# Human-Augment-Analytics/vectordb-retrieval

Measured on AMD Instinct MI355X. Metric: QPS @ recall@10 (SIFT1M-shaped, 10k-query batch, k=10), higher is better.
Workload: dtype i8 MFMA scan (i32 accumulate) + exact integer / f64 refine

## Files before the change

### vectordb-retrieval_amd/csrc/scan_i8x16.hpp

```cpp
#pragma once
#include "scan_i8.hpp"

namespace vdb {

__host__ __device__ inline int x16_row_in_span(int t, int rb, int m) { return (m >> 2) * 128 + t * 8 + rb * 4 + (m & 3); }

__device__ __forceinline__ int swap16(int v) { return __builtin_amdgcn_ds_swizzle(v, 0x401F); }

template <int KS2, int ST, int RING>
constexpr int scan_i8x16_lds_bytes() { return RING * (ST * 2 * KS2 * 64 * 16 + ST * 32 * 4); }

template <int N_MFMA, int N_VALU, int N_DS>
__device__ __forceinline__ void x16_gap_pattern() {
    constexpr int R = (N_VALU + N_DS + N_MFMA - 1) / N_MFMA;
    static_assert(N_DS <= N_MFMA && R >= 2, "one LDS read per gap");
#pragma unroll
    for (int i = 0; i < N_MFMA; ++i) {
        __builtin_amdgcn_sched_group_barrier(0x8, 1, 0);
        if (i < N_DS) {
            __builtin_amdgcn_sched_group_barrier(0x100, 1, 0);
            __builtin_amdgcn_sched_group_barrier(0x2, R - 1, 0);
        } else {
            __builtin_amdgcn_sched_group_barrier(0x2, R, 0);
        }
    }
}

template <int KS2, int ST, int CB, class StageIssue, class BiasStore, class FlushBin>
__device__ __forceinline__ void scan_i8x16_batch_loop(const unsigned char *smem, const int4v (&bq)[CB][KS2], int (&m1)[CB], int (&m2)[CB],
                                                      int nstages, int64_t span0, int lane, StageIssue &&stage_issue,
                                                      BiasStore &&stage_bias_store, FlushBin &&flush_bin) {
    constexpr int NV = 2 * KS2, kStageVec = ST * NV * 64, TPS = kTilesPerSpan, SPS = TPS / ST;
    constexpr int NM = 2 * KS2 * CB, NH = NM / 2;
    static_assert(ST % 2 == 0 && TPS % ST == 0, "tile parity must be static in the unrolled stage");
    const int g = lane >> 4;
    const unsigned id_hi = (g & 1) ? 16u : 0u;
    int4v acc[2][2][CB], fr[2][NV], cin[2][2];
    int q[CB];
#pragma unroll
    for (int rb = 0; rb < 2; ++rb)
#pragma unroll
        for (int cb = 0; cb < CB; ++cb)
#pragma unroll
            for (int r = 0; r < 4; ++r) acc[1][rb][cb][r] = (int)(kI8Inf >> 6);
    auto read_tile = [&](int p, const int4v *A, const int4v *B4, int t) {
#pragma unroll
        for (int v = 0; v < NV; ++v) fr[p][v] = A[(t * NV + v) * 64];
        cin[p][0] = B4[t * 8];
        cin[p][1] = B4[t * 8 + 1];
    };
    auto mfma_half = [&](int p, int half) {
#pragma unroll
        for (int m = half * NH; m < (half + 1) * NH; ++m) {
            const int ks = m / (2 * CB), rb = (m / CB) % 2, cb = m % CB;
            acc[p][rb][cb] = __builtin_amdgcn_mfma_i32_16x16x64_i8(fr[p][2 * ks + rb], bq[cb][ks], ks == 0 ? cin[p][rb] : acc[p][rb][cb], 0, 0, 0);
        }
    };
    auto min_trees = [&](int o) {
#pragma unroll
        for (int cb = 0; cb < CB; ++cb) {
            const int t1 = imin(imin(acc[o][0][cb][0], acc[o][0][cb][1]), acc[o][0][cb][2]);
            const int t2 = imin(imin(acc[o][0][cb][3], acc[o][1][cb][0]), acc[o][1][cb][1]);
            q[cb] = imin(imin(imin(acc[o][1][cb][2], acc[o][1][cb][3]), t1), t2);
        }
    };
    auto folds = [&](int t_bin) {
        const unsigned idv = (unsigned)__builtin_amdgcn_readfirstlane(t_bin) | id_hi;
#pragma unroll
        for (int cb = 0; cb < CB; ++cb) {
            const int v = (int)(((unsigned)q[cb] << 6) | idv);
            m2[cb] = imed3(m1[cb], m2[cb], v);
            m1[cb] = imin(m1[cb], v);
        }
    };
    for (int st = 0; st < nstages; ++st) {
        const int buf = st & 1;
        if (st + 1 < nstages) stage_issue(st + 1, buf ^ 1);
        const int4v *A = reinterpret_cast<const int4v *>(smem + buf * (kStageVec * 16)) + lane;
        const int4v *B4 = reinterpret_cast<const int4v *>(smem + 2 * kStageVec * 16 + buf * (ST * 32 * 4)) + g * 2;
        const int ts0 = (st % SPS) * ST;
        read_tile(0, A, B4, 0);
#pragma unroll
        for (int t = 0; t < ST; ++t) {
            const int p = t & 1, o = p ^ 1;
            __builtin_amdgcn_sched_barrier(0);
            mfma_half(p, 0);
            min_trees(o);
            x16_gap_pattern<NH, 4 * CB, 0>();
            __builtin_amdgcn_sched_barrier(0);
#pragma unroll
            for (int cb = 0; cb < CB; ++cb) asm volatile("" : "+v"(q[cb]));
            __builtin_amdgcn_sched_barrier(0);
            if (t + 1 < ST) read_tile(o, A, B4, t + 1);
            mfma_half(p, 1);
            folds((ts0 + t + TPS - 1) % TPS);
            x16_gap_pattern<NH, 3 * CB + 1, NV + 2>();
            __builtin_amdgcn_sched_barrier(0);
#pragma unroll
            for (int cb = 0; cb < CB; ++cb) asm volatile("" : "+v"(m1[cb]), "+v"(m2[cb]));
            if (t == 0 && st > 0 && ts0 == 0) flush_bin(span0 + st / SPS - 1);
        }
        __builtin_amdgcn_sched_barrier(0);
        if (st + 1 < nstages) stage_bias_store(buf ^ 1);
        __syncthreads();
    }
    min_trees((ST - 1) & 1);
    folds(TPS - 1);
    flush_bin(span0 + nstages / SPS - 1);
}

template <int KS2, int ST, int CB, int NWAVES = 8, int RING = 2, int AUX = 0>
__device__ __forceinline__ void scan_i8x16_body(const ScanI8Args &a, unsigned char *smem) {
    constexpr int NV = 2 * KS2;
    constexpr int NT = NWAVES * 64;
    constexpr int kStageVec = ST * NV * 64;
    constexpr int kBiasLoads = (ST * 32 + NT - 1) / NT;
    constexpr int TPS = kTilesPerSpan;
    constexpr int SPS = TPS / ST;
    constexpr int HC = CB / 2;
    constexpr int UNR = (ST * CB <= 16) ? ST : 1;
    static_assert(TPS % ST == 0 && ST >= 2 && CB % 2 == 0 && NWAVES <= 8, "bad geometry");
    static_assert(RING >= 2 && RING <= 8 && (RING == 2 || ST % 2 == 0), "bad ring");
    constexpr bool kDeep = RING > 2;
    static_assert(scan_i8x16_lds_bytes<KS2, ST, RING>() == RING * (kStageVec * 16 + ST * 32 * 4), "LDS size");
    const int mode = a.info->i8_mode;
    if (!mode) return;
    auto lds_a = [&](int buf) { return reinterpret_cast<int4v *>(smem + buf * (kStageVec * 16)); };
    auto lds_b = [&](int buf) { return reinterpret_cast<int *>(smem + RING * kStageVec * 16 + buf * (ST * 32 * 4)); };

    const int tid = threadIdx.x, lane = tid & 63;
    const int wave = __builtin_amdgcn_readfirstlane(tid >> 6);
    const int g = lane >> 4, h = g >> 1;
    const bool odd = (g & 1) != 0;
    const bool late = (NWAVES >= 2) && (wave >= NWAVES / 2);
    const int b = blockIdx.x;
    const int x = b & 7, jb = b >> 3;
    const int ci = jb / a.nqtiles, qt = jb - ci * a.nqtiles;
    const int chunk = x + 8 * ci;
    if (chunk >= a.nchunks) return;
    const int64_t q0 = (int64_t)qt * (NWAVES * 16 * CB) + wave * (16 * CB);
    const int64_t span0 = chunk_span0(chunk, a.spans_per_chunk, a.chunk_rem);
    int64_t span1 = chunk_span0(chunk + 1, a.spans_per_chunk, a.chunk_rem);
    if (span1 > a.nspans) span1 = a.nspans;
    const int64_t out_pitch = a.Qpad;
    const int64_t col0 = q0 + (odd ? 16 : 0) + (lane & 15);
    const int32_t *bias = a.bias8 + ((mode & 3) == 1 ? 0 : a.Npad);

    int4v bq[CB][KS2];
#pragma unroll
    for (int cb = 0; cb < CB; ++cb)
#pragma unroll
        for (int ks = 0; ks < KS2; ++ks) bq[cb][ks] = a.qpanels[((size_t)(q0 / 16 + cb) * KS2 + ks) * 64 + lane];
    const int nstages = (int)(span1 - span0) * SPS;
    const int INF = (int)kI8Inf;
    int m1[CB], m2[CB], M1[HC], M2[HC], Ms[HC];
#pragma unroll
    for (int cb = 0; cb < CB; ++cb) m1[cb] = m2[cb] = INF;
#pragma unroll
    for (int j = 0; j < HC; ++j) {
        M1[j] = M2[j] = INF;
        Ms[j] = 0;
    }

    constexpr int kPieces = kStageVec / 64;
    static_assert(kPieces % NWAVES == 0, "pieces must divide over the waves");
    constexpr int kBiasPieces = (ST / 2 + NWAVES - 1) / NWAVES;
    int stage_b[kBiasLoads];
    auto stage_issue = [&](int st, int buf) {
        const int64_t span = span0 + st / SPS;
        const int sq = st % SPS;
        const int4v *src = a.panels + ((size_t)(span * TPS + sq * ST) * NV) * 64;
        int4v *dst = lds_a(buf);
#pragma unroll
        for (int i = 0; i < kPieces / NWAVES; ++i) {
            const int p = wave + i * NWAVES;
            const int4v *gp = src + p * 64 + lane;
            __builtin_amdgcn_global_load_lds(
                reinterpret_cast<const __attribute__((address_space(1))) void *>(reinterpret_cast<uintptr_t>(gp)),
                reinterpret_cast<__attribute__((address_space(3))) void *>(
                    static_cast<uint32_t>(reinterpret_cast<uintptr_t>(dst + p * 64))),
                16, 0, AUX);
        }
        if (kDeep) {
#pragma unroll
            for (int i = 0; i < kBiasPieces; ++i) {
                const int j = (wave + i * NWAVES) % (ST / 2);
                const int t = 2 * j + (lane >> 5), gg = (lane >> 3) & 3, e = lane & 7;
                const int32_t *gp = bias + span * kSpanRows + gg * 128 + (sq * ST + t) * 8 + e;
                __builtin_amdgcn_global_load_lds(
                    reinterpret_cast<const __attribute__((address_space(1))) void *>(reinterpret_cast<uintptr_t>(gp)),
                    reinterpret_cast<__attribute__((address_space(3))) void *>(
                        static_cast<uint32_t>(reinterpret_cast<uintptr_t>(lds_b(buf) + j * 64))),
                    4, 0, 0);
            }
            return;
        }
#pragma unroll
        for (int i = 0; i < kBiasLoads; ++i) {
            const int e = tid + i * NT;
            if (e < ST * 32) {
                const int t = e >> 5, gg = (e >> 3) & 3, r = e & 7;
                stage_b[i] = bias[span * kSpanRows + gg * 128 + (sq * ST + t) * 8 + r];
            }
        }
    };
    auto stage_bias_store = [&](int buf) {
        if (kDeep) return;
#pragma unroll
        for (int i = 0; i < kBiasLoads; ++i)
            if (tid + i * NT < ST * 32) lds_b(buf)[tid + i * NT] = stage_b[i];
    };
    auto ring_issue = [&](int st) { stage_issue(st < nstages ? st : nstages - 1, st % RING); };
    auto ring_wait = [&]() {
        constexpr int kKeep = (RING - 2) * (kPieces / NWAVES + kBiasPieces);
        static_assert(kKeep < 64, "vmcnt is a 6-bit counter");
        asm volatile("s_waitcnt vmcnt(%0)" ::"n"(kKeep) : "memory");
        __builtin_amdgcn_s_barrier();
        asm volatile("" ::: "memory");
    };
    auto flush_bin = [&](int64_t span) {
        const size_t o = (size_t)(span * 2 + h) * out_pitch + col0;
#pragma unroll
        for (int j = 0; j < HC; ++j) {
            const int p1 = swap16(odd ? m1[2 * j] : m1[2 * j + 1]), p2 = swap16(odd ? m2[2 * j] : m2[2 * j + 1]);
            const int a1 = odd ? m1[2 * j + 1] : m1[2 * j], a2 = odd ? m2[2 * j + 1] : m2[2 * j];
            const int b1 = imin(a1, p1), b2 = imin(imax(a1, p1), imin(a2, p2));
            __builtin_nontemporal_store(__int_as_float(b1), a.bin_m1 + o + j * 32);
            __builtin_nontemporal_store(__int_as_float(b2), a.bin_m2 + o + j * 32);
            M2[j] = imin(imed3(M1[j], M2[j], b1), b2);
            if (b1 < M1[j]) Ms[j] = (int)span;
            M1[j] = imin(M1[j], b1);
        }
#pragma unroll
        for (int cb = 0; cb < CB; ++cb) m1[cb] = m2[cb] = INF;
    };

    if (kDeep) {
#pragma unroll
        for (int s = 0; s < RING - 1; ++s) ring_issue(s);
    } else {
        stage_issue(0, 0);
    }
    stage_bias_store(0);
    if (kDeep) ring_wait();
    else __syncthreads();

    if (a.nq_valid > 0 && q0 >= a.nq_valid) {
        for (int st = 0; st < nstages; ++st) {
            if (kDeep) {
                ring_issue(st + RING - 1);
                ring_wait();
                continue;
            }
            if (st + 1 < nstages) {
                stage_issue(st + 1, (st & 1) ^ 1);
                stage_bias_store((st & 1) ^ 1);
            }
            __syncthreads();
        }
        return;
    }

    if constexpr (NWAVES == 8 && RING == 2 && UNR == 1) {
        scan_i8x16_batch_loop<KS2, ST, CB>(smem, bq, m1, m2, nstages, span0, lane, stage_issue, stage_bias_store, flush_bin);
    } else {
    int4v fr[NV], cin[2], acc[2][CB];
    auto read_phase = [&](const int4v *A_tile, const int4v *c_tile) {
#pragma unroll
        for (int v = 0; v < NV; ++v) fr[v] = A_tile[v * 64 + lane];
        cin[0] = c_tile[0];
        cin[1] = c_tile[1];
    };
    auto mfma_phase = [&]() {
#pragma unroll
        for (int ks = 0; ks < KS2; ++ks)
#pragma unroll
            for (int rb = 0; rb < 2; ++rb)
#pragma unroll
                for (int cb = 0; cb < CB; ++cb)
                    acc[rb][cb] = __builtin_amdgcn_mfma_i32_16x16x64_i8(fr[2 * ks + rb], bq[cb][ks], ks == 0 ? cin[rb] : acc[rb][cb], 0, 0, 0);
    };
    const unsigned id_hi = odd ? 16u : 0u;
    auto select_phase = [&](int t_bin) {
        const unsigned idv = (unsigned)__builtin_amdgcn_readfirstlane(t_bin) | id_hi;
#pragma unroll
        for (int cb = 0; cb < CB; ++cb) {
            const int t1 = imin(imin(acc[0][cb][0], acc[0][cb][1]), acc[0][cb][2]);
            const int t2 = imin(imin(acc[0][cb][3], acc[1][cb][0]), acc[1][cb][1]);
            const int q = imin(imin(imin(acc[1][cb][2], acc[1][cb][3]), t1), t2);
            const int v = (int)(((unsigned)q << 6) | idv);
            m2[cb] = imed3(m1[cb], m2[cb], v);
            m1[cb] = imin(m1[cb], v);
        }
    };
    if (a.prio == 1 && late) __builtin_amdgcn_s_setprio(1);
    else if (a.prio == 2 && !late) __builtin_amdgcn_s_setprio(1);
    if (!late) {
        for (int st = 0; st < nstages; ++st) {
            const int buf = kDeep ? st % RING : st & 1;
            if (kDeep) ring_issue(st + RING - 1);
            else if (st + 1 < nstages) stage_issue(st + 1, buf ^ 1);
            const int4v *A = lds_a(buf);
            const int4v *B4 = reinterpret_cast<const int4v *>(lds_b(buf)) + g * 2;
            const int ts0 = (st % SPS) * ST;
            read_phase(A, B4);
#pragma unroll UNR
            for (int t = 0; t < ST; ++t) {
                __builtin_amdgcn_sched_barrier(0);
                mfma_phase();
                __builtin_amdgcn_sched_barrier(0);
                if (t + 1 < ST) read_phase(A + (t + 1) * NV * 64, B4 + (t + 1) * 8);
                select_phase(ts0 + t);
            }
            __builtin_amdgcn_sched_barrier(0);
            if (ts0 + ST == TPS) flush_bin(span0 + st / SPS);
            if (!kDeep && st + 1 < nstages) stage_bias_store(buf ^ 1);
            if (kDeep) ring_wait();
            else __syncthreads();
        }
    } else {
#pragma unroll
        for (int rb = 0; rb < 2; ++rb)
#pragma unroll
            for (int cb = 0; cb < CB; ++cb)
#pragma unroll
                for (int r = 0; r < 4; ++r) acc[rb][cb][r] = (int)(kI8Inf >> 6);
        for (int st = 0; st < nstages; ++st) {
            const int buf = kDeep ? st % RING : st & 1;
            if (kDeep) ring_issue(st + RING - 1);
            else if (st + 1 < nstages) stage_issue(st + 1, buf ^ 1);
            const int4v *A = lds_a(buf);
            const int4v *B4 = reinterpret_cast<const int4v *>(lds_b(buf)) + g * 2;
            const int ts0 = (st % SPS) * ST;
#pragma unroll UNR
            for (int t = 0; t < ST; ++t) {
                __builtin_amdgcn_sched_barrier(0);
                read_phase(A + t * NV * 64, B4 + t * 8);
                select_phase((ts0 + t + TPS - 1) % TPS);
                if (t == 0 && st > 0 && ts0 == 0) flush_bin(span0 + st / SPS - 1);
                __builtin_amdgcn_sched_barrier(0);
                mfma_phase();
            }
            __builtin_amdgcn_sched_barrier(0);
            if (!kDeep && st + 1 < nstages) stage_bias_store(buf ^ 1);
            if (kDeep) ring_wait();
            else __syncthreads();
        }
        select_phase(TPS - 1);
        flush_bin(span1 - 1);
    }
    }

    const size_t so = (size_t)(chunk * 2 + h) * a.Qpad + col0;
#pragma unroll
    for (int j = 0; j < HC; ++j) {
        a.sb_m1[so + j * 32] = __int_as_float(M1[j]);
        a.sb_m2[so + j * 32] = __int_as_float(M2[j]);
        a.sb_span[so + j * 32] = Ms[j];
    }
}

template <int KS2, int ST, int CB, int NWAVES = 8, int RING = 2, int AUX = 0>
__global__ __launch_bounds__(NWAVES * 64, (NWAVES >= 4 ? 2 : 1)) void scan_i8x16_kernel(ScanI8Args a) {
    __shared__ __attribute__((aligned(16))) unsigned char smem[scan_i8x16_lds_bytes<KS2, ST, RING>()];
    scan_i8x16_body<KS2, ST, CB, NWAVES, RING, AUX>(a, smem);
}

}
```

### vectordb-retrieval_amd/csrc/scan_x16.hpp

```cpp
#pragma once
#include "scan16.hpp"
#include "scan_i8x16.hpp"

namespace vdb {

template <int KS2, int ST>
constexpr int scan_x16_lds_bytes() { return 2 * (ST * 2 * KS2 * 64 * 16 + ST * 32 * 4); }

template <int KS2, int NWAVES, int ST, int BR = 256, int G = 8, int CB = 4>
__device__ __forceinline__ void scan_x16_body(const ScanArgs &a, unsigned char *smem) {
    constexpr int NV = 2 * KS2;
    static_assert(CB == 4 || (CB == 8 && KS2 <= 2), "128 queries per wave: D <= 64");
    constexpr int NT = NWAVES * 64;
    constexpr int kStageVec = ST * NV * 64;
    constexpr int kBiasLoads = (ST * 32 + NT - 1) / NT;
    constexpr int TPS = kTilesPerSpan;
    constexpr int SPS = TPS / ST;
    constexpr int BT = BR == 64 ? 8 : 16;
    constexpr bool kMerge = BR == 256;
    constexpr int NS = kMerge ? CB / 2 : CB;
    constexpr int UNR = ST <= 4 ? ST : 1;
    static_assert(TPS % ST == 0 && ST >= 2 && BT % ST == 0 && (BR == 256 || BR == 128 || BR == 64), "bad geometry");
    static_assert(G == 8 || (G == 4 && BR != 256), "quads: direct-bin mode");
    static_assert(scan_x16_lds_bytes<KS2, ST>() == 2 * (kStageVec * 16 + ST * 32 * 4), "LDS size");
    auto lds_a = [&](int buf) { return reinterpret_cast<half8 *>(smem + buf * (kStageVec * 16)); };
    auto lds_b = [&](int buf) { return reinterpret_cast<float *>(smem + 2 * kStageVec * 16 + buf * (ST * 32 * 4)); };
    if (a.info->i8_mode) return;

    const int tid = threadIdx.x, lane = tid & 63;
    const int wave = __builtin_amdgcn_readfirstlane(tid >> 6);
    const int g = lane >> 4, h = g >> 1;
    const bool odd = (g & 1) != 0;
    const bool late = (NWAVES >= 2) && (wave >= NWAVES / 2);
    const int b = blockIdx.x;
    const int x = b & 7, jb = b >> 3;
    const int ci = jb / a.nqtiles, qt = jb - ci * a.nqtiles;
    int chunk = x + 8 * ci;
    if (chunk >= a.nchunks) return;
    chunk += a.chunk0;
    const int64_t q0 = (int64_t)qt * (NWAVES * 16 * CB) + wave * (16 * CB);
    const int64_t span0 = chunk_span0(chunk, a.spans_per_chunk, a.chunk_rem);
    int64_t span1 = chunk_span0(chunk + 1, a.spans_per_chunk, a.chunk_rem);
    if (span1 > a.nspans) span1 = a.nspans;
    const int64_t col0 = q0 + ((kMerge && odd) ? 16 : 0) + (lane & 15);
    constexpr int CS = kMerge ? 32 : 16;
    const float cs = a.info->cs;

    half8 bq[CB][KS2];
#pragma unroll
    for (int cb = 0; cb < CB; ++cb)
#pragma unroll
        for (int ks = 0; ks < KS2; ++ks) bq[cb][ks] = a.qpanels[((size_t)(q0 / 16 + cb) * KS2 + ks) * 64 + lane];
    const int nstages = (int)(span1 - span0) * SPS;
    const float INF = __builtin_inff();
    float NEG_INF = -INF;
    asm volatile("" : "+v"(NEG_INF));
    unsigned idmask = kQuadIdMask;
    asm volatile("" : "+v"(idmask));
    float m1[CB], m2[CB], M1[NS], M2[NS];
    int Ms[NS];
#pragma unroll
    for (int cb = 0; cb < CB; ++cb) m1[cb] = m2[cb] = INF;
#pragma unroll
    for (int j = 0; j < NS; ++j) {
        M1[j] = M2[j] = INF;
        Ms[j] = 0;
    }

    constexpr int kPieces = kStageVec / 64;
    static_assert(kPieces % NWAVES == 0, "pieces must divide over the waves");
    float stage_b[kBiasLoads];
    auto stage_issue = [&](int st, int buf) {
        const int64_t span = span0 + st / SPS;
        const int sq = st % SPS;
        const half8 *src = a.panels + ((size_t)(span * TPS + sq * ST) * NV) * 64;
        half8 *dst = lds_a(buf);
#pragma unroll
        for (int i = 0; i < kPieces / NWAVES; ++i) {
            const int p = wave + i * NWAVES;
            const half8 *gp = src + p * 64 + lane;
            __builtin_amdgcn_global_load_lds(
                reinterpret_cast<const __attribute__((address_space(1))) void *>(reinterpret_cast<uintptr_t>(gp)),
                reinterpret_cast<__attribute__((address_space(3))) void *>(
                    static_cast<uint32_t>(reinterpret_cast<uintptr_t>(dst + p * 64))),
                16, 0, NWAVES <= 2 ? 2 : 0);
        }
#pragma unroll
        for (int i = 0; i < kBiasLoads; ++i) {
            const int e = tid + i * NT;
            if (e < ST * 32) {
                const int t = e >> 5, gg = (e >> 3) & 3, r = e & 7;
                stage_b[i] = a.bias[span * kSpanRows + gg * 128 + (sq * ST + t) * 8 + r];
            }
        }
    };
    auto stage_bias_store = [&](int buf) {
#pragma unroll
        for (int i = 0; i < kBiasLoads; ++i)
            if (tid + i * NT < ST * 32)
                lds_b(buf)[tid + i * NT] = (stage_b[i] >= 0.9e38f) ? kPadBias : stage_b[i] * cs;
    };
    auto flush_bin = [&](int64_t span, int bt) {
        if (kMerge) {
            const size_t o = (size_t)(span * 2 + h) * a.Qpad + col0;
#pragma unroll
            for (int j = 0; j < NS; ++j) {
                const float p1 = __int_as_float(swap16(__float_as_int(odd ? m1[2 * j] : m1[2 * j + 1])));
                const float p2 = __int_as_float(swap16(__float_as_int(odd ? m2[2 * j] : m2[2 * j + 1])));
                const float a1 = odd ? m1[2 * j + 1] : m1[2 * j], a2 = odd ? m2[2 * j + 1] : m2[2 * j];
                const float b1 = __builtin_fminf(a1, p1), b2 = __builtin_fminf(__builtin_fmaxf(a1, p1), __builtin_fminf(a2, p2));
                __builtin_nontemporal_store(b1, a.bin_m1 + o + j * CS);
                __builtin_nontemporal_store(b2, a.bin_m2 + o + j * CS);
                M2[j] = __builtin_fminf(__builtin_amdgcn_fmed3f(M1[j], M2[j], b1), b2);
                if (b1 < M1[j]) Ms[j] = (int)span;
                M1[j] = __builtin_fminf(M1[j], b1);
            }
        } else {
            const size_t o = (size_t)((span * 4 + g) * (128 / BR) + bt) * a.Qpad + col0;
#pragma unroll
            for (int j = 0; j < NS; ++j) {
                __builtin_nontemporal_store(m1[j], a.bin_m1 + o + j * 16);
                __builtin_nontemporal_store(m2[j], a.bin_m2 + o + j * 16);
                M2[j] = __builtin_fminf(__builtin_amdgcn_fmed3f(M1[j], M2[j], m1[j]), m2[j]);
                if (m1[j] < M1[j]) Ms[j] = (int)span;
                M1[j] = __builtin_fminf(M1[j], m1[j]);
            }
        }
#pragma unroll
        for (int cb = 0; cb < CB; ++cb) m1[cb] = m2[cb] = INF;
    };

    stage_issue(0, 0);
    stage_bias_store(0);
    __syncthreads();

    if (a.nq_valid > 0 && q0 >= a.nq_valid) {
        for (int st = 0; st < nstages; ++st) {
            if (st + 1 < nstages) {
                stage_issue(st + 1, (st & 1) ^ 1);
                stage_bias_store((st & 1) ^ 1);
            }
            __syncthreads();
        }
        return;
    }

    half8 fr[NV];
    float4v cin[2], acc[2][CB];
    auto read_phase = [&](const half8 *A_tile, const float4v *c_tile) {
#pragma unroll
        for (int v = 0; v < NV; ++v) fr[v] = A_tile[v * 64 + lane];
        cin[0] = c_tile[0];
        cin[1] = c_tile[1];
    };
    auto mfma_phase = [&]() {
#pragma unroll
        for (int ks = 0; ks < KS2; ++ks)
#pragma unroll
            for (int rb = 0; rb < 2; ++rb)
#pragma unroll
                for (int cb = 0; cb < CB; ++cb)
                    acc[rb][cb] = __builtin_amdgcn_mfma_f32_16x16x32_f16(fr[2 * ks + rb], bq[cb][ks], ks == 0 ? cin[rb] : acc[rb][cb], 0, 0, 0);
    };
    const unsigned id_hi = (kMerge && odd) ? 16u : 0u;
    auto select_phase = [&](int t_span) {
        const unsigned idv = (unsigned)__builtin_amdgcn_readfirstlane(t_span % BT) | id_hi;
#pragma unroll
        for (int cb = 0; cb < CB; ++cb) {
            if (G == 4) {
#pragma unroll
                for (int rb = 0; rb < 2; ++rb) {
                    const float qm = quad_min(acc[rb][cb][0], acc[rb][cb][1], acc[rb][cb][2], acc[rb][cb][3], NEG_INF);
                    const float v = pack_score(qm, idmask, 2u * idv + (unsigned)rb);
                    m2[cb] = __builtin_amdgcn_fmed3f(m1[cb], m2[cb], v);
                    m1[cb] = fast_min(m1[cb], v, NEG_INF);
                }
                continue;
            }
            const float o = oct_min(acc[0][cb][0], acc[0][cb][1], acc[0][cb][2], acc[0][cb][3], acc[1][cb][0], acc[1][cb][1],
                                    acc[1][cb][2], acc[1][cb][3], NEG_INF);
            const float v = pack_score(o, idmask, idv);
            m2[cb] = __builtin_amdgcn_fmed3f(m1[cb], m2[cb], v);
            m1[cb] = fast_min(m1[cb], v, NEG_INF);
        }
    };
    if (a.prio == 1 && late) __builtin_amdgcn_s_setprio(1);
    else if (a.prio == 2 && !late) __builtin_amdgcn_s_setprio(1);
    if (!late) {
        for (int st = 0; st < nstages; ++st) {
            const int buf = st & 1;
            if (st + 1 < nstages) stage_issue(st + 1, buf ^ 1);
            const half8 *A = lds_a(buf);
            const float4v *B4 = reinterpret_cast<const float4v *>(lds_b(buf)) + g * 2;
            const int ts0 = (st % SPS) * ST;
            read_phase(A, B4);
#pragma unroll UNR
            for (int t = 0; t < ST; ++t) {
                __builtin_amdgcn_sched_barrier(0);
                mfma_phase();
                __builtin_amdgcn_sched_barrier(0);
                if (t + 1 < ST) read_phase(A + (t + 1) * NV * 64, B4 + (t + 1) * 8);
                select_phase(ts0 + t);
            }
            __builtin_amdgcn_sched_barrier(0);
            if (((ts0 + ST) % BT) == 0) flush_bin(span0 + st / SPS, (ts0 + ST) / BT - 1);
            if (st + 1 < nstages) stage_bias_store(buf ^ 1);
            __syncthreads();
        }
    } else {
#pragma unroll
        for (int rb = 0; rb < 2; ++rb)
#pragma unroll
            for (int cb = 0; cb < CB; ++cb) acc[rb][cb] = float4v{3.0e38f, 3.0e38f, 3.0e38f, 3.0e38f};
        for (int st = 0; st < nstages; ++st) {
            const int buf = st & 1;
            if (st + 1 < nstages) stage_issue(st + 1, buf ^ 1);
            const half8 *A = lds_a(buf);
            const float4v *B4 = reinterpret_cast<const float4v *>(lds_b(buf)) + g * 2;
            const int ts0 = (st % SPS) * ST;
#pragma unroll UNR
            for (int t = 0; t < ST; ++t) {
                __builtin_amdgcn_sched_barrier(0);
                read_phase(A + t * NV * 64, B4 + t * 8);
                const int tp = (ts0 + t + TPS - 1) % TPS;
                select_phase(tp);
                if (t == 0 && st > 0 && (ts0 % BT) == 0) flush_bin(span0 + (st * ST - 1) / TPS, tp / BT);
                __builtin_amdgcn_sched_barrier(0);
                mfma_phase();
            }
            __builtin_amdgcn_sched_barrier(0);
            if (st + 1 < nstages) stage_bias_store(buf ^ 1);
            __syncthreads();
        }
        select_phase(TPS - 1);
        flush_bin(span1 - 1, TPS / BT - 1);
    }

    if (kMerge) {
        const size_t so = (size_t)(chunk * 2 + h) * a.Qpad + col0;
#pragma unroll
        for (int j = 0; j < NS; ++j) {
            a.sb_m1[so + j * CS] = M1[j];
            a.sb_m2[so + j * CS] = M2[j];
            a.sb_span[so + j * CS] = Ms[j];
        }
    }
}

template <int KS2, int NWAVES, int ST, int WPS, int BR = 256, int G = 8, int CB = 4>
__global__ __launch_bounds__(NWAVES * 64, WPS) void scan_x16_kernel(ScanArgs a) {
    __shared__ __attribute__((aligned(16))) unsigned char smem[scan_x16_lds_bytes<KS2, ST>()];
    scan_x16_body<KS2, NWAVES, ST, BR, G, CB>(a, smem);
}

template <bool W128, int NWAVES, int STF, int STI, int CBI, int RING, int AUX>
__global__ __launch_bounds__(NWAVES * 64, (NWAVES >= 4 ? 2 : 1)) void scan_pair_x16_kernel(ScanArgs a16, ScanI8Args a8) {
    constexpr int KF = W128 ? 4 : 2, KI = W128 ? 2 : 1;
    constexpr int kLds16 = scan_x16_lds_bytes<KF, STF>(), kLds8 = scan_i8x16_lds_bytes<KI, STI, RING>();
    __shared__ __attribute__((aligned(16))) unsigned char smem[kLds16 > kLds8 ? kLds16 : kLds8];
    if (a8.info->i8_mode) scan_i8x16_body<KI, STI, CBI, NWAVES, RING, AUX>(a8, smem);
    else scan_x16_body<KF, NWAVES, STF, 256>(a16, smem);
}

}
```

Measured before the change: 11.81 million.

## Use a three-buffer LDS ring in the i8 x16 batch loop to prefetch across barriers

The rolled 8-wave i8 scan loop moves from a two-buffer LDS double buffer to a three-buffer ring. The next stage's first tile can now be read before the barrier, and stage issue happens inside the first tile rather than before the stage. The separate bias-store step between stages is removed. This aims to hide LDS latency and global-to-LDS issue behind MFMA work, at the cost of one extra stage of LDS, which may reduce occupancy for these shapes.

```diff
diff --git a/vectordb-retrieval_amd/csrc/scan_i8x16.hpp b/vectordb-retrieval_amd/csrc/scan_i8x16.hpp
--- a/vectordb-retrieval_amd/csrc/scan_i8x16.hpp
+++ b/vectordb-retrieval_amd/csrc/scan_i8x16.hpp
@@ -1,5 +1,12 @@
 #pragma once
 #include "scan_i8.hpp"
+#include "scan_ring.hpp"
+
+#ifndef VDB_X16_STAMP
+#define VDB_X16_STAMP_BEGIN
+#define VDB_X16_STAMP(point) ((void)0)
+#define VDB_X16_STAMP_END
+#endif
 
 namespace vdb {
 
@@ -7,8 +14,8 @@
 
 __device__ __forceinline__ int swap16(int v) { return __builtin_amdgcn_ds_swizzle(v, 0x401F); }
 
-template <int KS2, int ST, int RING>
-constexpr int scan_i8x16_lds_bytes() { return RING * (ST * 2 * KS2 * 64 * 16 + ST * 32 * 4); }
+template <int KS2, int ST, int RING, int CB, int NWAVES>
+constexpr int scan_i8x16_lds_bytes() { return x16_lds_bytes(KS2, ST, CB, NWAVES, RING); }
 
 template <int N_MFMA, int N_VALU, int N_DS>
 __device__ __forceinline__ void x16_gap_pattern() {
@@ -26,13 +33,15 @@
     }
 }
 
-template <int KS2, int ST, int CB, class StageIssue, class BiasStore, class FlushBin>
+template <int KS2, int ST, int CB, class StageIssue, class FlushBin>
 __device__ __forceinline__ void scan_i8x16_batch_loop(const unsigned char *smem, const int4v (&bq)[CB][KS2], int (&m1)[CB], int (&m2)[CB],
                                                       int nstages, int64_t span0, int lane, StageIssue &&stage_issue,
-                                                      BiasStore &&stage_bias_store, FlushBin &&flush_bin) {
+                                                      FlushBin &&flush_bin) {
     constexpr int NV = 2 * KS2, kStageVec = ST * NV * 64, TPS = kTilesPerSpan, SPS = TPS / ST;
     constexpr int NM = 2 * KS2 * CB, NH = NM / 2;
+    constexpr int R = kX16BatchRing, kABytes = kStageVec * 16, kBBytes = ST * 32 * 4;
     static_assert(ST % 2 == 0 && TPS % ST == 0, "tile parity must be static in the unrolled stage");
+    static_assert(R >= 3, "a ring of 2 cannot read the next stage ahead of the barrier (scan_ring.hpp)");
     const int g = lane >> 4;
     const unsigned id_hi = (g & 1) ? 16u : 0u;
     int4v acc[2][2][CB], fr[2][NV], cin[2][2];
@@ -73,37 +82,54 @@
             m1[cb] = imin(m1[cb], v);
         }
     };
+    VDB_X16_STAMP_BEGIN
+    const unsigned char *pa = smem + lane * 16, *pb = smem + R * kABytes + g * 32;
+    int buf = 0;
+    read_tile(0, reinterpret_cast<const int4v *>(pa), reinterpret_cast<const int4v *>(pb), 0);
     for (int st = 0; st < nstages; ++st) {
-        const int buf = st & 1;
-        if (st + 1 < nstages) stage_issue(st + 1, buf ^ 1);
-        const int4v *A = reinterpret_cast<const int4v *>(smem + buf * (kStageVec * 16)) + lane;
-        const int4v *B4 = reinterpret_cast<const int4v *>(smem + 2 * kStageVec * 16 + buf * (ST * 32 * 4)) + g * 2;
+        const int nbuf = buf + 1 == R ? 0 : buf + 1, ibuf = nbuf + 1 == R ? 0 : nbuf + 1;
+        const int hop = ring_reads_ahead(st, nstages) ? nbuf - buf : 0;
+        const bool issue = ring_issues(st, nstages, R);
+        const int4v *A = reinterpret_cast<const int4v *>(pa), *B4 = reinterpret_cast<const int4v *>(pb);
         const int ts0 = (st % SPS) * ST;
-        read_tile(0, A, B4, 0);
+        const bool flush_due = st > 0 && ts0 == 0;
 #pragma unroll
         for (int t = 0; t < ST; ++t) {
             const int p = t & 1, o = p ^ 1;
             __builtin_amdgcn_sched_barrier(0);
+            if (t == 0) VDB_X16_STAMP(1);
             mfma_half(p, 0);
             min_trees(o);
             x16_gap_pattern<NH, 4 * CB, 0>();
             __builtin_amdgcn_sched_barrier(0);
 #pragma unroll
             for (int cb = 0; cb < CB; ++cb) asm volatile("" : "+v"(q[cb]));
+            if (t == ST - 1) {
+                pa += hop * kABytes;
+                pb += hop * kBBytes;
+            }
             __builtin_amdgcn_sched_barrier(0);
             if (t + 1 < ST) read_tile(o, A, B4, t + 1);
+            else read_tile(o, reinterpret_cast<const int4v *>(pa), reinterpret_cast<const int4v *>(pb), 0);
             mfma_half(p, 1);
             folds((ts0 + t + TPS - 1) % TPS);
             x16_gap_pattern<NH, 3 * CB + 1, NV + 2>();
             __builtin_amdgcn_sched_barrier(0);
 #pragma unroll
             for (int cb = 0; cb < CB; ++cb) asm volatile("" : "+v"(m1[cb]), "+v"(m2[cb]));
-            if (t == 0 && st > 0 && ts0 == 0) flush_bin(span0 + st / SPS - 1);
+            if (t == ST - 1) VDB_X16_STAMP(0);
+            if (t == 0 && issue) stage_issue(st + R - 1, ibuf);
+            if (t == 0 && flush_due) {
+                VDB_X16_STAMP(2);
+                flush_bin(span0 + st / SPS - 1);
+                VDB_X16_STAMP(3);
+            }
         }
         __builtin_amdgcn_sched_barrier(0);
-        if (st + 1 < nstages) stage_bias_store(buf ^ 1);
+        buf = nbuf;
         __syncthreads();
     }
+    VDB_X16_STAMP_END
     min_trees((ST - 1) & 1);
     folds(TPS - 1);
     flush_bin(span0 + nstages / SPS - 1);
@@ -121,12 +147,15 @@
     constexpr int UNR = (ST * CB <= 16) ? ST : 1;
     static_assert(TPS % ST == 0 && ST >= 2 && CB % 2 == 0 && NWAVES <= 8, "bad geometry");
     static_assert(RING >= 2 && RING <= 8 && (RING == 2 || ST % 2 == 0), "bad ring");
-    constexpr bool kDeep = RING > 2;
-    static_assert(scan_i8x16_lds_bytes<KS2, ST, RING>() == RING * (kStageVec * 16 + ST * 32 * 4), "LDS size");
+    constexpr bool kBatch = x16_batch_form(ST, CB, NWAVES, RING);
+    static_assert(kBatch == (NWAVES == 8 && RING == 2 && UNR == 1), "the batch forms are the rolled 8-wave shapes");
+    constexpr int NBUF = x16_ring_buffers(ST, CB, NWAVES, RING);
+    constexpr bool kDeep = NBUF > 2;
+    static_assert(scan_i8x16_lds_bytes<KS2, ST, RING, CB, NWAVES>() == NBUF * (kStageVec * 16 + ST * 32 * 4), "LDS size");
     const int mode = a.info->i8_mode;
     if (!mode) return;
     auto lds_a = [&](int buf) { return reinterpret_cast<int4v *>(smem + buf * (kStageVec * 16)); };
-    auto lds_b = [&](int buf) { return reinterpret_cast<int *>(smem + RING * kStageVec * 16 + buf * (ST * 32 * 4)); };
+    auto lds_b = [&](int buf) { return reinterpret_cast<int *>(smem + NBUF * kStageVec * 16 + buf * (ST * 32 * 4)); };
 
     const int tid = threadIdx.x, lane = tid & 63;
     const int wave = __builtin_amdgcn_readfirstlane(tid >> 6);
@@ -235,18 +264,28 @@
         for (int cb = 0; cb < CB; ++cb) m1[cb] = m2[cb] = INF;
     };
 
-    if (kDeep) {
+    if (kBatch) {
+#pragma unroll
+        for (int s = 0; s < kX16BatchRing - 1; ++s)
+            if (s < ring_prologue_stages(nstages, kX16BatchRing)) stage_issue(s, ring_buffer(s, kX16BatchRing));
+    } else if (kDeep) {
 #pragma unroll
         for (int s = 0; s < RING - 1; ++s) ring_issue(s);
     } else {
         stage_issue(0, 0);
     }
     stage_bias_store(0);
-    if (kDeep) ring_wait();
+    if (kDeep && !kBatch) ring_wait();
     else __syncthreads();
 
     if (a.nq_valid > 0 && q0 >= a.nq_valid) {
         for (int st = 0; st < nstages; ++st) {
+            if (kBatch) {
+                if (ring_issues(st, nstages, kX16BatchRing))
+                    stage_issue(ring_issue_stage(st, kX16BatchRing), ring_buffer(ring_issue_stage(st, kX16BatchRing), kX16BatchRing));
+                __syncthreads();
+                continue;
+            }
             if (kDeep) {
                 ring_issue(st + RING - 1);
                 ring_wait();
@@ -261,8 +300,8 @@
         return;
     }
 
-    if constexpr (NWAVES == 8 && RING == 2 && UNR == 1) {
-        scan_i8x16_batch_loop<KS2, ST, CB>(smem, bq, m1, m2, nstages, span0, lane, stage_issue, stage_bias_store, flush_bin);
+    if constexpr (kBatch) {
+        scan_i8x16_batch_loop<KS2, ST, CB>(smem, bq, m1, m2, nstages, span0, lane, stage_issue, flush_bin);
     } else {
     int4v fr[NV], cin[2], acc[2][CB];
     auto read_phase = [&](const int4v *A_tile, const int4v *c_tile) {
@@ -362,7 +401,7 @@
 
 template <int KS2, int ST, int CB, int NWAVES = 8, int RING = 2, int AUX = 0>
 __global__ __launch_bounds__(NWAVES * 64, (NWAVES >= 4 ? 2 : 1)) void scan_i8x16_kernel(ScanI8Args a) {
-    __shared__ __attribute__((aligned(16))) unsigned char smem[scan_i8x16_lds_bytes<KS2, ST, RING>()];
+    __shared__ __attribute__((aligned(16))) unsigned char smem[scan_i8x16_lds_bytes<KS2, ST, RING, CB, NWAVES>()];
     scan_i8x16_body<KS2, ST, CB, NWAVES, RING, AUX>(a, smem);
 }
 
diff --git a/vectordb-retrieval_amd/csrc/scan_ring.hpp b/vectordb-retrieval_amd/csrc/scan_ring.hpp
--- /dev/null
+++ b/vectordb-retrieval_amd/csrc/scan_ring.hpp
@@ -0,0 +1,26 @@
+#pragma once
+
+namespace vdb {
+
+constexpr int kX16BatchRing = 3;
+
+constexpr bool x16_batch_form(int st_tiles, int cb, int nwaves, int plan_ring) {
+    return nwaves == 8 && plan_ring == 2 && st_tiles * cb > 16;
+}
+constexpr int x16_ring_buffers(int st_tiles, int cb, int nwaves, int plan_ring) {
+    return x16_batch_form(st_tiles, cb, nwaves, plan_ring) ? kX16BatchRing : plan_ring;
+}
+constexpr int x16_stage_bytes(int ks2, int st_tiles) { return st_tiles * 2 * ks2 * 64 * 16 + st_tiles * 32 * 4; }
+constexpr int x16_lds_bytes(int ks2, int st_tiles, int cb, int nwaves, int plan_ring) {
+    return x16_ring_buffers(st_tiles, cb, nwaves, plan_ring) * x16_stage_bytes(ks2, st_tiles);
+}
+
+constexpr int ring_buffer(int s, int R) { return s % R; }
+constexpr int ring_prologue_stages(int nstages, int R) { return nstages < R - 1 ? nstages : R - 1; }
+constexpr int ring_issue_stage(int s, int R) { return s + R - 1; }
+constexpr bool ring_issues(int s, int nstages, int R) { return s + R - 1 < nstages; }
+constexpr int ring_certifier(int s, int R) { return s < R - 1 ? -1 : s - (R - 1); }
+constexpr bool ring_reads_ahead(int s, int nstages) { return s + 1 < nstages; }
+constexpr int ring_barriers(int nstages) { return nstages + 1; }
+
+}
diff --git a/vectordb-retrieval_amd/csrc/scan_x16.hpp b/vectordb-retrieval_amd/csrc/scan_x16.hpp
--- a/vectordb-retrieval_amd/csrc/scan_x16.hpp
+++ b/vectordb-retrieval_amd/csrc/scan_x16.hpp
@@ -256,7 +256,7 @@
 template <bool W128, int NWAVES, int STF, int STI, int CBI, int RING, int AUX>
 __global__ __launch_bounds__(NWAVES * 64, (NWAVES >= 4 ? 2 : 1)) void scan_pair_x16_kernel(ScanArgs a16, ScanI8Args a8) {
     constexpr int KF = W128 ? 4 : 2, KI = W128 ? 2 : 1;
-    constexpr int kLds16 = scan_x16_lds_bytes<KF, STF>(), kLds8 = scan_i8x16_lds_bytes<KI, STI, RING>();
+    constexpr int kLds16 = scan_x16_lds_bytes<KF, STF>(), kLds8 = scan_i8x16_lds_bytes<KI, STI, RING, CBI, NWAVES>();
     __shared__ __attribute__((aligned(16))) unsigned char smem[kLds16 > kLds8 ? kLds16 : kLds8];
     if (a8.info->i8_mode) scan_i8x16_body<KI, STI, CBI, NWAVES, RING, AUX>(a8, smem);
     else scan_x16_body<KF, NWAVES, STF, 256>(a16, smem);
```

Result: faster. 11.96 million, median of 6 (+1.3%).
